# hey-yahei/Quantization.MXNet

Hardware: AMD Instinct MI355X
Metric: images/sec int8-sim MobileNet1.0 (per-layer W8A8, online input quant) (higher is better)
Workload: dtype f32

## Files before the change

### quantization/mxnet_amd/csrc/fq_dw.h

```cpp
#ifndef FQ_DW_H_
#define FQ_DW_H_

#include "fq_common.h"

namespace fqi {

struct DwCall {
  const float *x, *w, *bias;
  float* y;
  int64_t n, c, h, wdt;
  int stride;
  const float *in_stat, *in_thr;
  float* out_current_max;
  const float *bn_scale, *bn_shift;
  int act;
  float* stat_out;
  hipStream_t st;
  bool quant, online, prezeroed;
  int epi;
  float levels, eps;
  int lo_neg;
  int64_t ho, wo;
  void* x_codes_out;
};

bool dw_flat_applies(const DwCall& d, int form), dw_planes_applies(const DwCall& d, int form);
bool dw_cols4_applies(const DwCall& d, int form), dw_cols_applies(const DwCall& d, int form);
bool dw_flat_stat_applies(const DwCall& d);
int dw_run_flat(const DwCall& d), dw_run_planes(const DwCall& d), dw_run_cols4(const DwCall& d), dw_run_cols(const DwCall& d);
int dw_run_tiles(const DwCall& d);
int dw_range_call(const float* x, const float* wcodes_f32, float* y, int64_t n, int64_t c, int64_t h, int64_t wdt, int stride,
                  const float* rec, const float* svec, const float* bn_scale, const float* bn_shift, int act,
                  float* stat_out, hipStream_t st);

}

namespace {

typedef float f2 __attribute__((ext_vector_type(2)));
__device__ __forceinline__ f2 splat2(float v) { return (f2){v, v}; }

__device__ __forceinline__ float dw_taps(float w00, float w01, float w02, float w10, float w11, float w12, float w20,
                                         float w21, float w22, float a0, float a1, float a2, float b0, float b1, float b2,
                                         float c0, float c1, float c2) {
  float acc = 0.0f;
  acc = fmaf(w00, a0, acc);
  acc = fmaf(w01, a1, acc);
  acc = fmaf(w02, a2, acc);
  acc = fmaf(w10, b0, acc);
  acc = fmaf(w11, b1, acc);
  acc = fmaf(w12, b2, acc);
  acc = fmaf(w20, c0, acc);
  acc = fmaf(w21, c1, acc);
  acc = fmaf(w22, c2, acc);
  return acc;
}
__device__ __forceinline__ f2 dw_taps2(float w00, float w01, float w02, float w10, float w11, float w12, float w20, float w21,
                                       float w22, f2 a0, f2 a1, f2 a2, f2 b0, f2 b1, f2 b2, f2 c0, f2 c1, f2 c2) {
  f2 acc = {0.f, 0.f};
  acc = __builtin_elementwise_fma(splat2(w00), a0, acc);
  acc = __builtin_elementwise_fma(splat2(w01), a1, acc);
  acc = __builtin_elementwise_fma(splat2(w02), a2, acc);
  acc = __builtin_elementwise_fma(splat2(w10), b0, acc);
  acc = __builtin_elementwise_fma(splat2(w11), b1, acc);
  acc = __builtin_elementwise_fma(splat2(w12), b2, acc);
  acc = __builtin_elementwise_fma(splat2(w20), c0, acc);
  acc = __builtin_elementwise_fma(splat2(w21), c1, acc);
  acc = __builtin_elementwise_fma(splat2(w22), c2, acc);
  return acc;
}

template <bool ONLINE>
__device__ __forceinline__ QParams dw_qparams(const float* in_stat, int n, const float* in_thr,
                                              float levels, int lo_neg_max, float eps, float* cur_max_out) {
  const float max_ = input_threshold(in_stat, n, ONLINE ? nullptr : in_thr, cur_max_out, blockIdx.x == 0);
  return make_qparams_rt(max_, levels, lo_neg_max, eps, in_thr);
}
template <bool ONLINE>
__device__ __forceinline__ QParams dw_qparams_finish(const ThresholdReq& treq, const float* in_stat, int n,
                                                     const float* in_thr, float levels, int lo_neg_max, float eps,
                                                     float* cur_max_out) {
  const float max_ = threshold_finish(treq, in_stat, n, ONLINE ? nullptr : in_thr, cur_max_out, blockIdx.x == 0);
  return make_qparams_rt(max_, levels, lo_neg_max, eps, in_thr);
}

struct DwBlkRange {
  unsigned begin, end;
  unsigned n_samples;
  unsigned s_base;
};
__device__ __forceinline__ DwBlkRange dw_block_range(unsigned nblk, unsigned tsegs, unsigned segs_per_block, unsigned nsegx,
                                                     unsigned C) {
  DwBlkRange r;
  r.begin = (unsigned)((uint64_t)nblk * blockIdx.x / gridDim.x);
  r.end = (unsigned)((uint64_t)nblk * (blockIdx.x + 1) / gridDim.x);
  r.n_samples = tsegs / nsegx / C;
  const unsigned seg0 = r.begin * segs_per_block;
  r.s_base = (seg0 < tsegs ? seg0 : tsegs - 1) / nsegx / C;
  return r;
}

constexpr int kDwStatSlots = 16;
template <class SampleT>
__device__ __forceinline__ void dw_stat_update(unsigned* k_stat, unsigned s_base, SampleT sample, bool is_out, float m,
                                               int lane, float* stat_out) {
  const unsigned s0 = (unsigned)__builtin_amdgcn_readfirstlane((int)sample);
  const bool wave_uniform = __all(!is_out || (unsigned)sample == s0);
  if (wave_uniform) {
    const float wm = wave_max_nonneg(is_out ? m : 0.0f);
    if (lane == 0 && __float_as_uint(wm) != 0u) {
      const unsigned slot = s0 - s_base;
      if (slot < (unsigned)kDwStatSlots) atomicMax(&k_stat[slot], __float_as_uint(wm));
      else atomic_max_f32(stat_out + s0, wm);
    }
  } else if (is_out) {
    const unsigned slot = (unsigned)sample - s_base;
    if (slot < (unsigned)kDwStatSlots) atomicMax(&k_stat[slot], __float_as_uint(m));
    else atomic_max_f32(stat_out + sample, m);
  }
}
__device__ __forceinline__ void dw_stat_flush(const unsigned* k_stat, unsigned s_base, unsigned n_samples,
                                              float* stat_out) {
  __syncthreads();
  if (threadIdx.x < kDwStatSlots && k_stat[threadIdx.x] != 0u && s_base + threadIdx.x < n_samples)
    FQ_STAT_FLUSH_MAX(reinterpret_cast<unsigned*>(stat_out) + s_base + threadIdx.x, k_stat[threadIdx.x]);
}

__device__ __forceinline__ float keep(float v, bool ok) { return __uint_as_float(__float_as_uint(v) & (ok ? 0xFFFFFFFFu : 0u)); }
__device__ __forceinline__ f4 keep4(f4 v, bool ok) {
  const unsigned mk = ok ? 0xFFFFFFFFu : 0u;
  f4 r;
  r.x = __uint_as_float(__float_as_uint(v.x) & mk);
  r.y = __uint_as_float(__float_as_uint(v.y) & mk);
  r.z = __uint_as_float(__float_as_uint(v.z) & mk);
  r.w = __uint_as_float(__float_as_uint(v.w) & mk);
  return r;
}
__device__ __forceinline__ float left_of(float v, bool first) {
  const float t = lane_prev(v);
  return first ? 0.0f : t;
}
__device__ __forceinline__ float right_of(float v, bool last) {
  const float t = lane_next(v);
  return last ? 0.0f : t;
}

struct DwColGeom {
  int C, H, W, Ho, Wo;
  int sw;
  int nsegx;
  int SEG;
  int segs;
  int nts;
};

__device__ __forceinline__ f2 buf_ld_2f32(fq_rsrc r, unsigned voff, unsigned soff) {
  return __builtin_bit_cast(f2, __builtin_amdgcn_raw_buffer_load_b64(r, (int)voff, (int)soff, 0));
}
__device__ __forceinline__ void buf_st_2f32(fq_rsrc r, unsigned voff, unsigned soff, f2 v) {
  typedef unsigned v2u __attribute__((ext_vector_type(2)));
  __builtin_amdgcn_raw_buffer_store_b64(__builtin_bit_cast(v2u, v), r, (int)voff, (int)soff, 0);
}

constexpr int kEpiRuntime = 0, kEpiBnRelu = 1, kEpiBnRelu6 = 2;
constexpr int kActBiasMul = 0x10;
template <int EPI, bool ACT = true>
__device__ __forceinline__ float dw_finish(float acc, bool has_bias, float bch, bool has_bn, float bsc, float bsh, int act) {
  if (EPI == kEpiRuntime) {
    if (has_bias) acc = (act & kActBiasMul) ? acc * bch : acc + bch;
    if (has_bn) {
      acc = acc * bsc;
      acc = acc + bsh;
    }
    return act_rt(acc, act & 15);
  }
  acc = acc * bsc;
  acc = acc + bsh;
  if (!ACT) return acc;
  acc = fmaxf(acc, 0.0f);
  return EPI == kEpiBnRelu6 ? fminf(acc, 6.0f) : acc;
}
template <int EPI>
__device__ __forceinline__ f2 dw_finish2(f2 acc, bool has_bias, float bch, bool has_bn, float bsc, float bsh, int act) {
  if (EPI == kEpiRuntime) {
    acc.x = dw_finish<EPI>(acc.x, has_bias, bch, has_bn, bsc, bsh, act);
    acc.y = dw_finish<EPI>(acc.y, has_bias, bch, has_bn, bsc, bsh, act);
    return acc;
  }
  acc = acc * splat2(bsc);
  acc = acc + splat2(bsh);
  acc.x = fmaxf(acc.x, 0.0f);
  acc.y = fmaxf(acc.y, 0.0f);
  if (EPI == kEpiBnRelu6) {
    acc.x = fminf(acc.x, 6.0f);
    acc.y = fminf(acc.y, 6.0f);
  }
  return acc;
}

constexpr unsigned kFlagRangeRecord = 0x100u;
constexpr unsigned kFlagBiasMultiplies = 0x200u;

template <class KernelFor, class... Geom>
int dw_launch(const DwCall& d, int grid, size_t lds, KernelFor kernel_for, Geom... geom) {
  using std::integral_constant;
  if (d.stat_out && !d.prezeroed) FQ_HIP(hipMemsetAsync(d.stat_out, 0, d.n * sizeof(float), d.st));
  const double in_bytes = 4.0 * (double)d.n * d.c * d.h * d.wdt, out_bytes = 4.0 * (double)d.n * d.c * d.ho * d.wo;
  ProfScope prof(FQ_KERNEL_DWCONV, in_bytes + out_bytes, d.st,
                 d.y ? -1.0 : in_bytes + (d.x_codes_out ? 0.25 * in_bytes : 0.0));
  float* const y_arg = d.y ? d.y : static_cast<float*>(d.x_codes_out);
  auto launch = [&](auto kernel) {
    hipLaunchKernelGGL(kernel, dim3(grid), dim3(kBlock), lds, d.st, d.x, d.w, d.bias, y_arg, geom..., d.in_stat, (int)d.n,
                       d.in_thr, d.levels, d.lo_neg, d.eps, d.out_current_max, d.bn_scale, d.bn_shift, d.act, d.stat_out);
  };
  auto with_epi = [&](auto quant_c, auto online_c) {
    if (d.epi == kEpiBnRelu) launch(kernel_for(quant_c, online_c, integral_constant<int, kEpiBnRelu>{}));
    else if (d.epi == kEpiBnRelu6) launch(kernel_for(quant_c, online_c, integral_constant<int, kEpiBnRelu6>{}));
    else launch(kernel_for(quant_c, online_c, integral_constant<int, kEpiRuntime>{}));
  };
  if (!d.quant) with_epi(std::false_type{}, std::false_type{});
  else if (d.online) with_epi(std::true_type{}, std::true_type{});
  else with_epi(std::true_type{}, std::false_type{});
  FQ_LAUNCH_CHECK();
  return FQ_OK;
}
template <int V>
using dw_int = std::integral_constant<int, V>;

inline int64_t dw_blocks(int64_t total_segs, int segs) {
  const int64_t per_block = (int64_t)segs * (kBlock / 64);
  return (total_segs + per_block - 1) / per_block;
}
inline int dw_grid(int64_t nblk, int wg_per_cu) {
  const int64_t cap = (int64_t)num_cu() * wg_per_cu;
  return (int)(nblk < cap ? nblk : cap);
}

inline DwColGeom dw_col_geom(const DwCall& d, int units, int halo) {
  DwColGeom cg = {};
  cg.C = (int)d.c;
  cg.H = (int)d.h;
  cg.W = (int)d.wdt;
  cg.Ho = (int)d.ho;
  cg.Wo = (int)d.wo;
  const int max_sw = 64 - halo;
  cg.nsegx = (units + max_sw - 1) / max_sw;
  cg.sw = (units + cg.nsegx - 1) / cg.nsegx;
  cg.SEG = cg.sw + halo;
  cg.segs = 64 / cg.SEG;
  return cg;
}
inline int dw_cols_grid(int64_t total_segs, const DwColGeom& cg) {
  static const int dw_wg_per_cu = env_int("FQ_DW_WG_PER_CU", 6);
  return dw_grid(dw_blocks(total_segs, cg.segs), dw_wg_per_cu);
}

}

#endif
```

### quantization/mxnet_amd/csrc/fq_dw_cols.hip

```cpp
#include "fq_dw.h"

namespace {
template <int S, bool QUANT, bool ONLINE, int EPI>
__global__ __launch_bounds__(kBlock) void dwconv3x3_cols_kernel(
    const float* __restrict__ x, const float* __restrict__ wgt, const float* __restrict__ bias,
    float* __restrict__ y, DwColGeom g, int64_t total_segs, const float* __restrict__ in_stat, int n,
    const float* __restrict__ in_thr, float levels, int lo_neg_max, float eps, float* __restrict__ cur_max_out,
    const float* __restrict__ bn_scale, const float* __restrict__ bn_shift, int act, float* __restrict__ stat_out) {
  constexpr int D = (S == 1) ? 8 : 4;
  __shared__ unsigned k_stat[kDwStatSlots];
  if (threadIdx.x < kDwStatSlots) k_stat[threadIdx.x] = 0u;
  PW_STAMP(0);
  QParams q = {};
  bool q_ready = !QUANT;
  auto ensure_q = [&]() __attribute__((always_inline)) {
    if (QUANT && !q_ready) {
      q = dw_qparams<ONLINE>(in_stat, n, in_thr, levels, lo_neg_max, eps, cur_max_out);
      q_ready = true;
    }
  };
  PW_STAMP(1);
  const int lane = threadIdx.x & 63, wave = threadIdx.x >> 6;
  const int seg_in_wave = lane / g.SEG;
  const int pos = lane - seg_in_wave * g.SEG;
  const bool lane_used = seg_in_wave < g.segs;
  const int64_t segs_per_block = (int64_t)g.segs * (kBlock / 64);
  const int64_t nblk = (total_segs + segs_per_block - 1) / segs_per_block;
  const bool has_bn = bn_scale != nullptr, has_stat = stat_out != nullptr;
  const int plane_in = g.H * g.W, plane_out = g.Ho * g.Wo;

  const unsigned tsegs = (unsigned)total_segs, nsegx = (unsigned)g.nsegx, C_u = (unsigned)g.C;
  const DwBlkRange rg = dw_block_range((unsigned)nblk, tsegs, (unsigned)segs_per_block, nsegx, C_u);
  __syncthreads();
  for (unsigned blk = rg.begin; blk < rg.end; ++blk) {
    const unsigned seg = blk * (unsigned)segs_per_block + (unsigned)wave * (unsigned)g.segs + (unsigned)seg_in_wave;
    const bool seg_ok = lane_used && seg < tsegs;
    const unsigned plane = seg_ok ? seg / nsegx : 0u;
    const int sx = seg_ok ? (int)(seg - plane * nsegx) : 0;
    const unsigned sample_u = plane / C_u;
    const int ch = (int)(plane - sample_u * C_u);
    const int sample = (int)sample_u;
    int oc, ic0;
    bool is_out;
    if (S == 1) {
      ic0 = sx * g.sw + pos - 1;
      oc = ic0;
      is_out = seg_ok && pos >= 1 && pos <= g.sw && oc < g.Wo;
    } else {
      oc = sx * g.sw + pos - 1;
      ic0 = 2 * oc;
      is_out = seg_ok && pos >= 1 && oc < g.Wo;
    }
    const bool ld0 = seg_ok && (S == 1 ? (ic0 >= 0 && ic0 < g.W) : (pos >= 1 && ic0 < g.W));
    const bool ld1 = seg_ok && S == 2 && (ic0 + 1 >= 0) && (ic0 + 1 < g.W);
    const float* xp = x + plane * (int64_t)plane_in + ic0;
    float* yp = y + plane * (int64_t)plane_out + oc;
    const float* wk = wgt + ch * 9;
    const float w00 = wk[0], w01 = wk[1], w02 = wk[2], w10 = wk[3], w11 = wk[4], w12 = wk[5], w20 = wk[6],
                w21 = wk[7], w22 = wk[8];
    const float bch = bias != nullptr ? bias[ch] : 0.0f;
    const float bsc = has_bn ? bn_scale[ch] : 1.0f, bsh = has_bn ? bn_shift[ch] : 0.0f;
    float m = 0.0f;
    if (blk == rg.begin) PW_STAMP(2);

    const int last_row = g.H - 1;
    if (S == 1) {
      const float* xs = ld0 ? xp : x;
      auto ldrow = [&](int row) -> float {
        const int rc = row < last_row ? row : last_row;
        return keep(xs[(int64_t)rc * g.W], ld0 && row <= last_row);
      };
      auto emit = [&](int r, float c1, float& a0, float& a1, float& a2, float& b0, float& b1, float& b2) {
        if (QUANT) c1 = fq_code(c1, q) * q.scale;
        const float c0 = lane_prev(c1), c2 = lane_next(c1);
        float acc = dw_taps(w00, w01, w02, w10, w11, w12, w20, w21, w22, a0, a1, a2, b0, b1, b2, c0, c1, c2);
        acc = dw_finish<EPI>(acc, bias != nullptr, bch, has_bn, bsc, bsh, act);
        m = fmaxf(m, keep(fabsf(acc), is_out));
        if (is_out) yp[(int64_t)r * g.Wo] = acc;
        a0 = b0; a1 = b1; a2 = b2;
        b0 = c0; b1 = c1; b2 = c2;
      };
      float raw[D];
#pragma unroll
      for (int k = 0; k < D; ++k) raw[k] = ldrow(1 + k);
      float a0 = 0.f, a1 = 0.f, a2 = 0.f;
      float b1 = ldrow(0);
      FQ_PIN();
      ensure_q();
      if (QUANT) b1 = fq_code(b1, q) * q.scale;
      float b0 = lane_prev(b1), b2 = lane_next(b1);
      const int rend = g.Ho;
      int r0 = 0;
      for (; r0 + D <= rend; r0 += D) {
#pragma unroll
        for (int k = 0; k < D; ++k) {
          const float c1 = raw[k];
          raw[k] = ldrow(r0 + k + 1 + D);
          emit(r0 + k, c1, a0, a1, a2, b0, b1, b2);
        }
      }
#pragma unroll
      for (int k = 0; k < D; ++k)
        if (r0 + k < rend) emit(r0 + k, raw[k], a0, a1, a2, b0, b1, b2);
    } else {
      const float* xs0 = ld0 ? xp : x;
      const float* xs1 = ld1 ? xp + 1 : x;
      auto ld_a = [&](int row) -> float {
        const int rc = row < last_row ? row : last_row;
        return keep(xs0[(int64_t)rc * g.W], ld0 && row <= last_row);
      };
      auto ld_b = [&](int row) -> float {
        const int rc = row < last_row ? row : last_row;
        return keep(xs1[(int64_t)rc * g.W], ld1 && row <= last_row);
      };
      auto emit2 = [&](int r, float b1, float b2, float c1, float c2, float& a0, float& a1, float& a2) {
        if (QUANT) {
          b1 = fq_code(b1, q) * q.scale;
          b2 = fq_code(b2, q) * q.scale;
          c1 = fq_code(c1, q) * q.scale;
          c2 = fq_code(c2, q) * q.scale;
        }
        const float b0 = lane_prev(b2), c0 = lane_prev(c2);
        float acc = dw_taps(w00, w01, w02, w10, w11, w12, w20, w21, w22, a0, a1, a2, b0, b1, b2, c0, c1, c2);
        acc = dw_finish<EPI>(acc, bias != nullptr, bch, has_bn, bsc, bsh, act);
        m = fmaxf(m, keep(fabsf(acc), is_out));
        if (is_out) yp[(int64_t)r * g.Wo] = acc;
        a0 = c0; a1 = c1; a2 = c2;
      };
      float rb0[D], rb1[D], rc0[D], rc1[D];
#pragma unroll
      for (int k = 0; k < D; ++k) {
        rb0[k] = ld_a(2 * k);
        rb1[k] = ld_b(2 * k);
        rc0[k] = ld_a(2 * k + 1);
        rc1[k] = ld_b(2 * k + 1);
      }
      FQ_PIN();
      ensure_q();
      float a0 = 0.f, a1 = 0.f, a2 = 0.f;
      const int rend = g.Ho;
      int r0 = 0;
      for (; r0 + D <= rend; r0 += D) {
#pragma unroll
        for (int k = 0; k < D; ++k) {
          const float b1 = rb0[k], b2 = rb1[k], c1 = rc0[k], c2 = rc1[k];
          const int rn = r0 + k + D;
          rb0[k] = ld_a(2 * rn);
          rb1[k] = ld_b(2 * rn);
          rc0[k] = ld_a(2 * rn + 1);
          rc1[k] = ld_b(2 * rn + 1);
          emit2(r0 + k, b1, b2, c1, c2, a0, a1, a2);
        }
      }
#pragma unroll
      for (int k = 0; k < D; ++k)
        if (r0 + k < rend) emit2(r0 + k, rb0[k], rb1[k], rc0[k], rc1[k], a0, a1, a2);
    }
    if (blk == rg.begin) PW_STAMP(3);
    if (has_stat) dw_stat_update(k_stat, rg.s_base, sample, is_out, m, lane, stat_out);
  }
  if (has_stat) dw_stat_flush(k_stat, rg.s_base, rg.n_samples, stat_out);
  PW_STAMP(5);
}

template <int S, bool QUANT, bool ONLINE, bool NT, int EPI, bool NOSTORE = false>
__global__ __launch_bounds__(kBlock) void dwconv3x3_cols4_kernel(
    const float* __restrict__ x, const float* __restrict__ wgt, const float* __restrict__ bias,
    float* __restrict__ y, DwColGeom g, int64_t total_segs, const float* __restrict__ in_stat, int n,
    const float* __restrict__ in_thr, float levels, int lo_neg_max, float eps, float* __restrict__ cur_max_out,
    const float* __restrict__ bn_scale, const float* __restrict__ bn_shift, int act, float* __restrict__ stat_out) {
  constexpr int D = (S == 1) ? 4 : 2;
  static_assert(!NOSTORE || (S == 1 && QUANT), "the statistic pass exists for stride 1 with a quantised input");
  __shared__ unsigned k_stat[kDwStatSlots];
  if (threadIdx.x < kDwStatSlots) k_stat[threadIdx.x] = 0u;
  QParams q = {};
  if (QUANT) q = dw_qparams<ONLINE>(in_stat, n, in_thr, levels, lo_neg_max, eps, cur_max_out);
  const int lane = threadIdx.x & 63, wave = threadIdx.x >> 6;
  const int seg_in_wave = lane / g.SEG;
  const int pos = lane - seg_in_wave * g.SEG;
  const bool lane_used = seg_in_wave < g.segs;
  const int64_t segs_per_block = (int64_t)g.segs * (kBlock / 64);
  const int64_t nblk = (total_segs + segs_per_block - 1) / segs_per_block;
  const bool has_bn = bn_scale != nullptr, has_stat = stat_out != nullptr;
  const int plane_in = g.H * g.W, plane_out = g.Ho * g.Wo;
  const int last_row = g.H - 1;
  const unsigned tsegs = (unsigned)total_segs, nsegx = (unsigned)g.nsegx, C_u = (unsigned)g.C;
  const DwBlkRange rg = dw_block_range((unsigned)nblk, tsegs, (unsigned)segs_per_block, nsegx, C_u);
  __syncthreads();
  for (unsigned blk = rg.begin; blk < rg.end; ++blk) {
    const unsigned seg = blk * (unsigned)segs_per_block + (unsigned)wave * (unsigned)g.segs + (unsigned)seg_in_wave;
    const bool seg_ok = lane_used && seg < tsegs;
    const unsigned plane = seg_ok ? seg / nsegx : 0u;
    const int sx = seg_ok ? (int)(seg - plane * nsegx) : 0;
    const unsigned sample_u = plane / C_u;
    const int ch = (int)(plane - sample_u * C_u);
    const int sample = (int)sample_u;
    const int ic0 = (sx * g.sw + pos - 1) * 4;
    const bool ld_ok = seg_ok && ic0 >= 0 && ic0 < g.W;
    const int oc = S == 1 ? ic0 : ic0 / 2;
    const bool is_out = seg_ok && pos >= 1 && pos <= g.sw && oc < g.Wo;
    const f4* xs = reinterpret_cast<const f4*>(ld_ok ? x + plane * (int64_t)plane_in + ic0 : x);
    float* yp = y + plane * (int64_t)plane_out + oc;
    const int rowq = g.W / 4;
    const float* wk = wgt + ch * 9;
    const float w00 = wk[0], w01 = wk[1], w02 = wk[2], w10 = wk[3], w11 = wk[4], w12 = wk[5], w20 = wk[6],
                w21 = wk[7], w22 = wk[8];
    const float bch = bias != nullptr ? bias[ch] : 0.0f;
    const float bsc = has_bn ? bn_scale[ch] : 1.0f, bsh = has_bn ? bn_shift[ch] : 0.0f;
    float m = 0.0f;
    auto ldrow = [&](int row) -> f4 {
      const int rc = row < last_row ? row : last_row;
      return keep4(ld4<NT>(xs + (int64_t)rc * rowq), ld_ok && row <= last_row);
    };
    auto quant4 = [&](f4 v) -> f4 { return QUANT ? fq_code4(v, q) * q.scale : v; };
    auto finish = [&](float acc) -> float { return dw_finish<EPI>(acc, bias != nullptr, bch, has_bn, bsc, bsh, act); };
    unsigned* const cp = reinterpret_cast<unsigned*>(y) + (plane * (int64_t)plane_in + (ld_ok ? ic0 : 0)) / 4;
    auto quant4_keep = [&](f4 v, int row) -> f4 {
      const f4 k = fq_code4(v, q);
      if (y != nullptr && is_out && row <= last_row) {
        const unsigned b0 = (unsigned)(int)k.x & 255u, b1 = (unsigned)(int)k.y & 255u, b2 = (unsigned)(int)k.z & 255u,
                       b3 = (unsigned)(int)k.w & 255u;
        cp[(int64_t)row * rowq] = b0 | (b1 << 8) | (b2 << 16) | (b3 << 24);
      }
      return k * q.scale;
    };

    if (S == 1) {
      float a[6] = {0.f, 0.f, 0.f, 0.f, 0.f, 0.f}, b[6];
      f4 raw[D];
#pragma unroll
      for (int k = 0; k < D; ++k) raw[k] = ldrow(1 + k);
      {
        const f4 v = NOSTORE ? quant4_keep(ldrow(0), 0) : quant4(ldrow(0));
        b[0] = lane_prev(v.w);
        b[1] = v.x; b[2] = v.y; b[3] = v.z; b[4] = v.w;
        b[5] = lane_next(v.x);
      }
      auto emit = [&](int r, f4 craw) {
        const f4 v = NOSTORE ? quant4_keep(craw, r + 1) : quant4(craw);
        float c[6];
        c[0] = lane_prev(v.w);
        c[1] = v.x; c[2] = v.y; c[3] = v.z; c[4] = v.w;
        c[5] = lane_next(v.x);
        float o[4];
#pragma unroll
        for (int k = 0; k < 4; ++k) {
          o[k] = finish(dw_taps(w00, w01, w02, w10, w11, w12, w20, w21, w22, a[k], a[k + 1], a[k + 2], b[k], b[k + 1],
                                b[k + 2], c[k], c[k + 1], c[k + 2]));
        }
        const float mm = fmaxf(fmaxf(fabsf(o[0]), fabsf(o[1])), fmaxf(fabsf(o[2]), fabsf(o[3])));
        m = fmaxf(m, keep(mm, is_out));
        if (!NOSTORE && is_out) {
          if (g.nts) __builtin_nontemporal_store((f4){o[0], o[1], o[2], o[3]}, reinterpret_cast<f4*>(yp + (int64_t)r * g.Wo));
          else *reinterpret_cast<f4*>(yp + (int64_t)r * g.Wo) = (f4){o[0], o[1], o[2], o[3]};
        }
#pragma unroll
        for (int k = 0; k < 6; ++k) {
          a[k] = b[k];
          b[k] = c[k];
        }
      };
      int r0 = 0;
      for (; r0 + D <= g.Ho; r0 += D) {
        f4 nxt[D];
#pragma unroll
        for (int k = 0; k < D; ++k) nxt[k] = ldrow(r0 + k + 1 + D);
#pragma unroll
        for (int k = 0; k < D; ++k) emit(r0 + k, raw[k]);
#pragma unroll
        for (int k = 0; k < D; ++k) raw[k] = nxt[k];
      }
#pragma unroll
      for (int k = 0; k < D; ++k)
        if (r0 + k < g.Ho) emit(r0 + k, raw[k]);
    } else {
      float a[5] = {0.f, 0.f, 0.f, 0.f, 0.f};
      f4 rb[D], rc[D];
#pragma unroll
      for (int k = 0; k < D; ++k) {
        rb[k] = ldrow(2 * k);
        rc[k] = ldrow(2 * k + 1);
      }
      auto emit2 = [&](int r, f4 braw, f4 craw) {
        const f4 vb = quant4(braw), vc = quant4(craw);
        const float b[5] = {lane_prev(vb.w), vb.x, vb.y, vb.z, vb.w};
        const float c[5] = {lane_prev(vc.w), vc.x, vc.y, vc.z, vc.w};
        float o[2];
#pragma unroll
        for (int k = 0; k < 2; ++k) {
          o[k] = finish(dw_taps(w00, w01, w02, w10, w11, w12, w20, w21, w22, a[2 * k], a[2 * k + 1], a[2 * k + 2], b[2 * k],
                                b[2 * k + 1], b[2 * k + 2], c[2 * k], c[2 * k + 1], c[2 * k + 2]));
        }
        m = fmaxf(m, keep(fmaxf(fabsf(o[0]), fabsf(o[1])), is_out));
        if (is_out) {
          typedef float f2v __attribute__((ext_vector_type(2)));
          if (g.nts) __builtin_nontemporal_store((f2v){o[0], o[1]}, reinterpret_cast<f2v*>(yp + (int64_t)r * g.Wo));
          else *reinterpret_cast<float2*>(yp + (int64_t)r * g.Wo) = make_float2(o[0], o[1]);
        }
#pragma unroll
        for (int k = 0; k < 5; ++k) a[k] = c[k];
      };
      int r0 = 0;
      for (; r0 + D <= g.Ho; r0 += D) {
        f4 nb[D], nc[D];
#pragma unroll
        for (int k = 0; k < D; ++k) {
          nb[k] = ldrow(2 * (r0 + k + D));
          nc[k] = ldrow(2 * (r0 + k + D) + 1);
        }
#pragma unroll
        for (int k = 0; k < D; ++k) emit2(r0 + k, rb[k], rc[k]);
#pragma unroll
        for (int k = 0; k < D; ++k) {
          rb[k] = nb[k];
          rc[k] = nc[k];
        }
      }
#pragma unroll
      for (int k = 0; k < D; ++k)
        if (r0 + k < g.Ho) emit2(r0 + k, rb[k], rc[k]);
    }
    if (has_stat) dw_stat_update(k_stat, rg.s_base, sample, is_out, m, lane, stat_out);
  }
  if (has_stat) dw_stat_flush(k_stat, rg.s_base, rg.n_samples, stat_out);
}

}

namespace fqi {
bool dw_cols4_applies(const DwCall& d, int form) {
  const bool can4 = (d.wdt % 4 == 0) && aligned16(d.x) && aligned16(d.y) && aligned16(d.x_codes_out) && ((d.h * d.wdt) % 4 == 0) &&
                    (d.stride == 1 || ((d.wdt / 2) % 2 == 0));
  return (form == 3 || form == 0) && can4;
}
int dw_run_cols4(const DwCall& d) {
  DwColGeom cg = dw_col_geom(d, (int)(d.wdt / 4), d.stride == 1 ? 2 : 1);
  const int64_t total_segs = d.n * d.c * cg.nsegx;
  FQ_REQUIRE(total_segs < (1ll << 31) - 1024, "fq_dwconv3x3: tensor too large for 32-bit segment indices");
  const int grid = dw_cols_grid(total_segs, cg);
  static const int dw_nt_mb = env_int("FQ_DW_NT_MB", 200);
  const bool nt = 4.0 * (double)d.n * d.c * d.h * d.wdt > 1e6 * dw_nt_mb;
  static const int dw_nts_mb = env_int("FQ_DW_NTS_MB", 1 << 30);
  cg.nts = 4.0 * (double)d.n * d.c * cg.Ho * cg.Wo >= 1e6 * dw_nts_mb ? 1 : 0;
  auto go = [&](auto s, auto nt_c) {
    return dw_launch(d, grid, 0, [](auto q, auto o, auto e) {
      return dwconv3x3_cols4_kernel<decltype(s)::value, q(), o(), decltype(nt_c)::value, e()>;
    }, cg, total_segs);
  };
  if (d.y == nullptr) {
    auto go_stat = [&](auto nt_c) {
      return dw_launch(d, grid, 0, [](auto, auto o, auto e) {
        return dwconv3x3_cols4_kernel<1, true, o(), decltype(nt_c)::value, e(), true>;
      }, cg, total_segs);
    };
    return nt ? go_stat(std::true_type{}) : go_stat(std::false_type{});
  }
  if (d.stride == 1) return nt ? go(dw_int<1>{}, std::true_type{}) : go(dw_int<1>{}, std::false_type{});
  return nt ? go(dw_int<2>{}, std::true_type{}) : go(dw_int<2>{}, std::false_type{});
}
bool dw_cols_applies(const DwCall& d, int form) {
  return form == 2 || ((form == 0 || form == 3) && d.wdt >= 14);
}
int dw_run_cols(const DwCall& d) {
  const DwColGeom cg = dw_col_geom(d, (int)d.wo, d.stride == 1 ? 2 : 1);
  const int64_t total_segs = d.n * d.c * cg.nsegx;
  FQ_REQUIRE(total_segs < (1ll << 31) - 1024, "fq_dwconv3x3: tensor too large for 32-bit segment indices");
  const int grid = dw_cols_grid(total_segs, cg);
  auto go = [&](auto s) {
    return dw_launch(d, grid, 0, [](auto q, auto o, auto e) {
      return dwconv3x3_cols_kernel<decltype(s)::value, q(), o(), e()>;
    }, cg, total_segs);
  };
  return d.stride == 1 ? go(dw_int<1>{}) : go(dw_int<2>{});
}
}
```

### quantization/mxnet_amd/csrc/fq_dw_flat.hip

```cpp
#include "fq_dw.h"

namespace {
#define FQ_DWF_PHASE()                                             \
  do {                                                             \
    __builtin_amdgcn_fence(__ATOMIC_RELEASE, "wavefront");         \
    __builtin_amdgcn_wave_barrier();                               \
    __builtin_amdgcn_fence(__ATOMIC_ACQUIRE, "wavefront");         \
  } while (0)

struct DwFlatGeom {
  int C;
  unsigned planes;
  unsigned per, rem;
  FastDiv by_c;
};

template <int S, bool QUANT, bool ONLINE, int H, int W, int EPI>
__global__ __launch_bounds__(kBlock) void dwconv3x3_flat_kernel(
    const float* __restrict__ x, const float* __restrict__ wgt, const float* __restrict__ bias,
    float* __restrict__ y, DwFlatGeom g, const float* __restrict__ in_stat, int n, const float* __restrict__ in_thr,
    float levels, int lo_neg_max, float eps, float* __restrict__ cur_max_out, const float* __restrict__ bn_scale,
    const float* __restrict__ bn_shift, int act, float* __restrict__ stat_out) {
  constexpr bool PAIR = S == 1 && W % 2 == 0, DOWN = S == 2;
  static_assert(S == 1 || W % 2 == 0, "stride 2 reads column pairs");
// ... 117 lines not shown
        }
      } else {
        auto window = [&](float a0, float a1, float a2, float b0, float b1, float b2, float c0, float c1, float c2) -> float {
          float acc = dw_taps(w03.x, w03.y, w03.z, w03.w, w47.x, w47.y, w47.z, w47.w, cur.w8, a0, a1, a2, b0, b1, b2, c0, c1, c2);
          acc = dw_finish<EPI>(acc, has_bias, cur.bch, has_bn, cur.bsc, cur.bsh, act);
          m = fmaxf(m, fabsf(acc));
          return acc;
        };
        if (!DOWN) {
          float* lp = my_tile + j * IN + pos;
          float a0 = 0.f, a1 = 0.f, a2 = 0.f;
          float b1 = lp[0];
          float b0 = left_of(b1, first), b2 = right_of(b1, last);
#pragma unroll
          for (int r = 0; r < H; ++r) {
            float c0 = 0.f, c1 = 0.f, c2 = 0.f;
            if (r + 1 < H) {
              c1 = lp[(r + 1) * W];
              c0 = left_of(c1, first);
              c2 = right_of(c1, last);
            }
            lp[r * W] = window(a0, a1, a2, b0, b1, b2, c0, c1, c2);
            a0 = b0; a1 = b1; a2 = b2;
            b0 = c0; b1 = c1; b2 = c2;
          }
        } else {
          const float* lp = my_tile + j * IN + pos * 2;
          float* op = my_out + j * OUT + pos;
          float a0 = 0.f, a1 = 0.f, a2 = 0.f;
#pragma unroll
          for (int r = 0; r < HO; ++r) {
            const f2 vb = *reinterpret_cast<const f2*>(lp + (2 * r) * W);
            const float b0 = left_of(vb.y, first);
            float c0 = 0.f, c1 = 0.f, c2 = 0.f;
            if (2 * r + 1 < H) {
              const f2 vc = *reinterpret_cast<const f2*>(lp + (2 * r + 1) * W);
              c1 = vc.x;
              c2 = vc.y;
              c0 = left_of(vc.y, first);
            }
            op[r * WO] = window(a0, a1, a2, b0, vb.x, vb.y, c0, c1, c2);
            a0 = c0; a1 = c1; a2 = c2;
          }
        }
      }
    }
    FQ_DWF_PHASE();
    {
      f4 ov[NLO];
#pragma unroll
      for (int i = 0; i < NLO; ++i) ov[i] = DOWN ? otile[wave][lane + 64 * i] : tile[wave][lane + 64 * i];
#pragma unroll
      for (int i = 0; i < NLO; ++i)
        buf_st_v4f_unguarded(ry, (lane + 64u * i) < lim_out ? lane * 16u : kOob, base * (OUT * 4u) + 1024u * i, ov[i]);
      hold_store_data(ov);
    }
    if (has_stat) {
      const unsigned sample = fast_div(base + (is_out ? j : 0u), g.by_c);
      dw_stat_update(k_stat, s_base, sample, is_out, m, (int)lane, stat_out);
    }
    __builtin_amdgcn_wave_barrier();
  }
  PW_STAMP(3);
  if (has_stat) dw_stat_flush(k_stat, s_base, n_samples, stat_out);
  PW_STAMP(5);
}

template <bool ONLINE, int H, int W, int EPI>
__global__ __launch_bounds__(kBlock) void dwconv3x3_flat_stat_kernel(
    const float* __restrict__ x, const float* __restrict__ wgt, const float* __restrict__ bias,
    float* __restrict__ y, DwFlatGeom g, const float* __restrict__ in_stat, int n, const float* __restrict__ in_thr,
    float levels, int lo_neg_max, float eps, float* __restrict__ cur_max_out, const float* __restrict__ bn_scale,
    const float* __restrict__ bn_shift, int act, float* __restrict__ stat_out) {
  static_assert(W % 2 == 0 && (H * W) % 4 == 0, "two columns per lane, planes of whole 16-byte groups");
  constexpr int IN = H * W;
  constexpr int LPP = W / 2;
  constexpr int P = 64 / LPP;
  constexpr int NFI = P * IN / 4;
  constexpr int NLI = (NFI + 63) / 64;
  constexpr unsigned kOob = 0x80000000u;
  __shared__ f4 tile[kBlock / 64][NLI * 64];
  __shared__ unsigned k_stat[kDwStatSlots];
  if (threadIdx.x < kDwStatSlots) k_stat[threadIdx.x] = 0u;
  const unsigned lane = threadIdx.x & 63u;
  const unsigned wave = (unsigned)__builtin_amdgcn_readfirstlane((int)(threadIdx.x >> 6));
  const unsigned b = blockIdx.x;
  const unsigned blk_begin = b * g.per + (b < g.rem ? b : g.rem);
  const unsigned blk_end = blk_begin + g.per + (b < g.rem ? 1u : 0u);
  const unsigned planes = g.planes;
  const unsigned n_samples = (unsigned)n;
  unsigned s_base;
  {
    const unsigned p0 = blk_begin * (P * (kBlock / 64));
    s_base = fast_div(p0 < planes ? p0 : planes - 1, g.by_c);
  }
  const bool has_bn = bn_scale != nullptr, has_stat = stat_out != nullptr, has_bias = bias != nullptr;
  const fq_rsrc rx = make_rsrc(x, (int64_t)planes * IN * 4), rc = make_rsrc(y, y != nullptr ? (int64_t)planes * IN : 0);
  const fq_rsrc rw = make_rsrc(wgt, (int64_t)g.C * 36);
  const unsigned j = lane / LPP, pos = lane - j * LPP;
  const bool b_lane = lane < P * LPP;
  const bool first = pos == 0, last = pos == LPP - 1;
  float* const my_tile = reinterpret_cast<float*>(tile[wave]);

  struct Blk {
    f4 raw[NLI];
    f4 w03, w47;
    float w8, bch, bsc, bsh;
  };
  auto issue = [&](unsigned blk, Blk& k) __attribute__((always_inline)) {
    const unsigned base = (blk * (kBlock / 64) + wave) * P;
    const unsigned left = base < planes ? planes - base : 0u;
    const unsigned np = left < (unsigned)P ? left : (unsigned)P;
    const unsigned lim = np * (IN / 4);
#pragma unroll
    for (int i = 0; i < NLI; ++i)
      k.raw[i] = buf_ld_v4f_nt(rx, (lane + 64u * i) < lim ? lane * 16u : kOob, base * (IN * 4u) + 1024u * i);
    const unsigned ch = (b_lane && j < left) ? fast_mod(base + j, g.by_c) : 0u;
    k.w03 = buf_ld_v4f(rw, ch * 36u, 0);
    k.w47 = buf_ld_v4f(rw, ch * 36u, 16);
    k.w8 = buf_ld_f32(rw, ch * 36u, 32);
    k.bch = has_bias ? bias[ch] : 0.0f;
    k.bsc = has_bn ? bn_scale[ch] : 1.0f;
    k.bsh = has_bn ? bn_shift[ch] : 0.0f;
  };

  Blk nxt;
  const ThresholdReq treq = threshold_request(in_stat, n, ONLINE ? nullptr : in_thr, blockIdx.x == 0);
  FQ_PIN();
  if (blk_begin < blk_end) issue(blk_begin, nxt);
  FQ_PIN();
  const QParams q = dw_qparams_finish<ONLINE>(treq, in_stat, n, in_thr, levels, lo_neg_max, eps, cur_max_out);
  __syncthreads();
  for (unsigned blk = blk_begin; blk < blk_end; ++blk) {
    Blk cur = nxt;
    FQ_PIN();
    if (blk + 1 < blk_end) issue(blk + 1, nxt);
    FQ_PIN();
    const unsigned base = (blk * (kBlock / 64) + wave) * P;
    const unsigned left = base < planes ? planes - base : 0u;
    const unsigned np = left < (unsigned)P ? left : (unsigned)P;
    const unsigned lim = np * (IN / 4);
#pragma unroll
    for (int i = 0; i < NLI; ++i) {
      const f4 k = fq_code4(cur.raw[i], q);
      const unsigned wd = ((unsigned)(int)k.x & 255u) | (((unsigned)(int)k.y & 255u) << 8) | (((unsigned)(int)k.z & 255u) << 16) |
                          (((unsigned)(int)k.w & 255u) << 24);
      buf_st_f32(rc, (lane + 64u * i) < lim ? lane * 4u : kOob, base * (unsigned)IN + 256u * i, __uint_as_float(wd));
      tile[wave][lane + 64 * i] = k * q.scale;
    }
    FQ_DWF_PHASE();
    float m = 0.0f;
    const bool is_out = b_lane && j < left;
    if (b_lane) {
      const f4 w03 = cur.w03, w47 = cur.w47;
      const float* lp = my_tile + j * IN + pos * 2;
      f2 aL = {0.f, 0.f}, aC = {0.f, 0.f}, aR = {0.f, 0.f};
      f2 bL, bC, bR;
      {
        const f2 v = *reinterpret_cast<const f2*>(lp);
        bL = (f2){left_of(v.y, first), v.x};
        bC = v;
        bR = (f2){v.y, right_of(v.x, last)};
      }
#pragma unroll
      for (int r = 0; r < H; ++r) {
        f2 cL = {0.f, 0.f}, cC = {0.f, 0.f}, cR = {0.f, 0.f};
        if (r + 1 < H) {
          const f2 v = *reinterpret_cast<const f2*>(lp + (r + 1) * W);
          cL = (f2){left_of(v.y, first), v.x};
          cC = v;
          cR = (f2){v.y, right_of(v.x, last)};
        }
        f2 acc = dw_taps2(w03.x, w03.y, w03.z, w03.w, w47.x, w47.y, w47.z, w47.w, cur.w8, aL, aC, aR, bL, bC, bR, cL, cC, cR);
        acc = dw_finish2<EPI>(acc, has_bias, cur.bch, has_bn, cur.bsc, cur.bsh, act);
        m = fmaxf(m, fmaxf(fabsf(acc.x), fabsf(acc.y)));
        aL = bL; aC = bC; aR = bR;
        bL = cL; bC = cC; bR = cR;
      }
    }
    if (has_stat) {
      const unsigned sample = fast_div(base + (is_out ? j : 0u), g.by_c);
      dw_stat_update(k_stat, s_base, sample, is_out, m, (int)lane, stat_out);
    }
    FQ_DWF_PHASE();
  }
  if (has_stat) dw_stat_flush(k_stat, s_base, n_samples, stat_out);
}

int dw_flat_kind(const DwCall& d) {
  return (d.h == 14 && d.wdt == 14) ? (d.stride == 1 ? 0 : 1)
         : (d.h == 7 && d.wdt == 7 && d.stride == 1) ? 2
         : (d.h == 28 && d.wdt == 28) ? (d.stride == 1 ? 3 : 4) : -1;
}
int dw_flat_planes(int kind) { return kind == 0 ? 9 : kind >= 3 ? 4 : 8; }

}

namespace fqi {
bool dw_flat_applies(const DwCall& d, int form) {
  static const int flat_on = env_int("FQ_DW_FLAT", 31) & 31;
  const int kind = dw_flat_kind(d);
  const bool whole = kind == 0 || kind >= 3 || (d.n * d.c) % dw_flat_planes(kind) == 0;
  return kind >= 0 && (form == 5 || (form == 0 && ((flat_on >> kind) & 1))) && whole && aligned16(d.x) && aligned16(d.y) &&
         d.n * d.c * d.h * d.wdt * 4 < (1ll << 31);
}
bool dw_flat_stat_applies(const DwCall& d) {
  static const int flat_on = env_int("FQ_DW_FLAT", 31) & 31;
  return d.y == nullptr && d.quant && d.lo_neg != kRangeMode && dw_flat_kind(d) == 3 && ((flat_on >> 3) & 1) && aligned16(d.x) &&
         aligned16(d.x_codes_out) && d.n * d.c * d.h * d.wdt * 4 < (1ll << 31);
}
int dw_run_flat(const DwCall& d) {
  const int kind = dw_flat_kind(d);
  DwFlatGeom fg;
  fg.C = (int)d.c;
  fg.planes = (unsigned)(d.n * d.c);
  fg.by_c = fast_div_for((unsigned)d.c);
  const int64_t nblk = dw_blocks(d.n * d.c, dw_flat_planes(kind));
  static const int fl_tune = env_int("FQ_DW_FLAT_WG_PER_CU", 0);
  const int grid = dw_grid(nblk, fl_tune > 0 ? fl_tune : 3);
  fg.per = (unsigned)(nblk / grid);
  fg.rem = (unsigned)(nblk % grid);
  if (d.y == nullptr)
    return dw_launch(d, grid, 0, [](auto, auto o, auto e) { return dwconv3x3_flat_stat_kernel<o(), 28, 28, e()>; }, fg);
  auto go = [&](auto s, auto hw) {
    return dw_launch(d, grid, 0, [](auto q, auto o, auto e) {
      return dwconv3x3_flat_kernel<decltype(s)::value, q(), o(), decltype(hw)::value, decltype(hw)::value, e()>;
    }, fg);
  };
  return kind == 0 ? go(dw_int<1>{}, dw_int<14>{}) : kind == 1 ? go(dw_int<2>{}, dw_int<14>{})
         : kind == 2 ? go(dw_int<1>{}, dw_int<7>{}) : kind == 4 ? go(dw_int<2>{}, dw_int<28>{})
                     : go(dw_int<1>{}, dw_int<28>{});
}
}
```

Before: 170,100.

## Split depthwise statistic pass into row strips and defer epilogue to min/max

Adds a dedicated statistic kernel for the depthwise conv that only computes the output abs-max. It splits each column block into row strips so small-batch or small-grid layers expose more work units per CU. It also tracks raw accumulator min/max and applies the bias/BN/activation epilogue only to those two values instead of every output, in both the cols and flat kernels. A fast non-negative quantisation path using a reciprocal quotient is added. The costs are halo rows reloaded per strip and reliance on the epilogue being monotonic so the min/max shortcut stays exact.

```diff
diff --git a/quantization/mxnet_amd/csrc/fq_dw.h b/quantization/mxnet_amd/csrc/fq_dw.h
--- a/quantization/mxnet_amd/csrc/fq_dw.h
+++ b/quantization/mxnet_amd/csrc/fq_dw.h
@@ -2,6 +2,7 @@
 #define FQ_DW_H_
 
 #include "fq_common.h"
+#include "fq_dw_strips.h"
 
 namespace fqi {
 
@@ -250,9 +251,23 @@
   cg.segs = 64 / cg.SEG;
   return cg;
 }
+inline int dw_cols_wg_per_cu() {
+  static const int dw_wg_per_cu = env_int("FQ_DW_WG_PER_CU", 6);
+  return dw_wg_per_cu;
+}
 inline int dw_cols_grid(int64_t total_segs, const DwColGeom& cg) {
-  static const int dw_wg_per_cu = env_int("FQ_DW_WG_PER_CU", 6);
-  return dw_grid(dw_blocks(total_segs, cg.segs), dw_wg_per_cu);
+  return dw_grid(dw_blocks(total_segs, cg.segs), dw_cols_wg_per_cu());
+}
+struct DwStatGeom {
+  int strips;
+  FastDiv by_strips;
+};
+inline DwStatGeom dw_stat_geom(int64_t total_segs, const DwColGeom& cg) {
+  const char* e = getenv("FQ_DW_STAT_STRIPS");
+  DwStatGeom sg;
+  sg.strips = dw_stat_strips(dw_blocks(total_segs, cg.segs), cg.H, num_cu(), e != nullptr ? atoi(e) : 0);
+  sg.by_strips = fast_div_for((unsigned)sg.strips);
+  return sg;
 }
 
 }
diff --git a/quantization/mxnet_amd/csrc/fq_dw_cols.hip b/quantization/mxnet_amd/csrc/fq_dw_cols.hip
--- a/quantization/mxnet_amd/csrc/fq_dw_cols.hip
+++ b/quantization/mxnet_amd/csrc/fq_dw_cols.hip
@@ -170,7 +170,7 @@
     const float* __restrict__ in_thr, float levels, int lo_neg_max, float eps, float* __restrict__ cur_max_out,
     const float* __restrict__ bn_scale, const float* __restrict__ bn_shift, int act, float* __restrict__ stat_out) {
   constexpr int D = (S == 1) ? 4 : 2;
-  static_assert(!NOSTORE || (S == 1 && QUANT), "the statistic pass exists for stride 1 with a quantised input");
+  static_assert(!NOSTORE, "the statistic pass is dwconv3x3_cols4_stat_kernel");
   __shared__ unsigned k_stat[kDwStatSlots];
   if (threadIdx.x < kDwStatSlots) k_stat[threadIdx.x] = 0u;
   QParams q = {};
@@ -214,16 +214,6 @@
     };
     auto quant4 = [&](f4 v) -> f4 { return QUANT ? fq_code4(v, q) * q.scale : v; };
     auto finish = [&](float acc) -> float { return dw_finish<EPI>(acc, bias != nullptr, bch, has_bn, bsc, bsh, act); };
-    unsigned* const cp = reinterpret_cast<unsigned*>(y) + (plane * (int64_t)plane_in + (ld_ok ? ic0 : 0)) / 4;
-    auto quant4_keep = [&](f4 v, int row) -> f4 {
-      const f4 k = fq_code4(v, q);
-      if (y != nullptr && is_out && row <= last_row) {
-        const unsigned b0 = (unsigned)(int)k.x & 255u, b1 = (unsigned)(int)k.y & 255u, b2 = (unsigned)(int)k.z & 255u,
-                       b3 = (unsigned)(int)k.w & 255u;
-        cp[(int64_t)row * rowq] = b0 | (b1 << 8) | (b2 << 16) | (b3 << 24);
-      }
-      return k * q.scale;
-    };
 
     if (S == 1) {
       float a[6] = {0.f, 0.f, 0.f, 0.f, 0.f, 0.f}, b[6];
@@ -231,13 +221,13 @@
 #pragma unroll
       for (int k = 0; k < D; ++k) raw[k] = ldrow(1 + k);
       {
-        const f4 v = NOSTORE ? quant4_keep(ldrow(0), 0) : quant4(ldrow(0));
+        const f4 v = quant4(ldrow(0));
         b[0] = lane_prev(v.w);
         b[1] = v.x; b[2] = v.y; b[3] = v.z; b[4] = v.w;
         b[5] = lane_next(v.x);
       }
       auto emit = [&](int r, f4 craw) {
-        const f4 v = NOSTORE ? quant4_keep(craw, r + 1) : quant4(craw);
+        const f4 v = quant4(craw);
         float c[6];
         c[0] = lane_prev(v.w);
         c[1] = v.x; c[2] = v.y; c[3] = v.z; c[4] = v.w;
@@ -250,7 +240,7 @@
         }
         const float mm = fmaxf(fmaxf(fabsf(o[0]), fabsf(o[1])), fmaxf(fabsf(o[2]), fabsf(o[3])));
         m = fmaxf(m, keep(mm, is_out));
-        if (!NOSTORE && is_out) {
+        if (is_out) {
           if (g.nts) __builtin_nontemporal_store((f4){o[0], o[1], o[2], o[3]}, reinterpret_cast<f4*>(yp + (int64_t)r * g.Wo));
           else *reinterpret_cast<f4*>(yp + (int64_t)r * g.Wo) = (f4){o[0], o[1], o[2], o[3]};
         }
@@ -323,6 +313,146 @@
     if (has_stat) dw_stat_update(k_stat, rg.s_base, sample, is_out, m, lane, stat_out);
   }
   if (has_stat) dw_stat_flush(k_stat, rg.s_base, rg.n_samples, stat_out);
+}
+
+template <bool ONLINE, bool NT, int EPI>
+__global__ __launch_bounds__(kBlock) void dwconv3x3_cols4_stat_kernel(
+    const float* __restrict__ x, const float* __restrict__ wgt, const float* __restrict__ bias,
+    float* __restrict__ y, DwColGeom g, int64_t total_segs, DwStatGeom sg, const float* __restrict__ in_stat, int n,
+    const float* __restrict__ in_thr, float levels, int lo_neg_max, float eps, float* __restrict__ cur_max_out,
+    const float* __restrict__ bn_scale, const float* __restrict__ bn_shift, int act, float* __restrict__ stat_out) {
+  constexpr int D = kDwStatBurst;
+  __shared__ unsigned k_stat[kDwStatSlots];
+  if (threadIdx.x < kDwStatSlots) k_stat[threadIdx.x] = 0u;
+  const QParams q = dw_qparams<ONLINE>(in_stat, n, in_thr, levels, lo_neg_max, eps, cur_max_out);
+  const FastQuot fqx = make_fast_quot(q.denom);
+  const bool fast = fq_nonneg(q) && fqx.ok;
+  const int lane = threadIdx.x & 63, wave = threadIdx.x >> 6;
+  const int seg_in_wave = lane / g.SEG;
+  const int pos = lane - seg_in_wave * g.SEG;
+  const bool lane_used = seg_in_wave < g.segs;
+  const unsigned segs_per_block = (unsigned)g.segs * (kBlock / 64);
+  const bool has_bn = bn_scale != nullptr, has_stat = stat_out != nullptr;
+  const int plane_in = g.H * g.W;
+  const int last_row = g.H - 1;
+  const int rowq = g.W / 4;
+  const unsigned tsegs = (unsigned)total_segs, nsegx = (unsigned)g.nsegx, C_u = (unsigned)g.C;
+  const int64_t units = (int64_t)((tsegs + segs_per_block - 1) / segs_per_block) * sg.strips;
+  const unsigned u_begin = (unsigned)dw_stat_unit_begin(units, (int)gridDim.x, (int)blockIdx.x);
+  const unsigned u_end = (unsigned)dw_stat_unit_begin(units, (int)gridDim.x, (int)blockIdx.x + 1);
+  const unsigned n_samples = tsegs / nsegx / C_u;
+  unsigned s_base;
+  {
+    const unsigned seg0 = fast_div(u_begin, sg.by_strips) * segs_per_block;
+    s_base = (seg0 < tsegs ? seg0 : tsegs - 1) / nsegx / C_u;
+  }
+  __syncthreads();
+  auto walk = [&](auto fast_c) __attribute__((always_inline)) {
+    constexpr bool FAST = decltype(fast_c)::value;
+    for (unsigned unit = u_begin; unit < u_end; ++unit) {
+      const unsigned blk = fast_div(unit, sg.by_strips);
+      const DwStrip strip = dw_stat_strip(g.H, sg.strips, (int)(unit - blk * (unsigned)sg.strips));
+      const int r_begin = strip.r0, r_end = strip.r0 + strip.rows;
+      const unsigned seg = blk * segs_per_block + (unsigned)wave * (unsigned)g.segs + (unsigned)seg_in_wave;
+      const bool seg_ok = lane_used && seg < tsegs;
+      const unsigned plane = seg_ok ? seg / nsegx : 0u;
+      const int sx = seg_ok ? (int)(seg - plane * nsegx) : 0;
+      const unsigned sample_u = plane / C_u;
+      const int ch = (int)(plane - sample_u * C_u);
+      const int sample = (int)sample_u;
+      const int ic0 = (sx * g.sw + pos - 1) * 4;
+      const bool ld_ok = seg_ok && ic0 >= 0 && ic0 < g.W;
+      const bool is_out = seg_ok && pos >= 1 && pos <= g.sw && ic0 < g.W;
+      const f4* xs = reinterpret_cast<const f4*>(ld_ok ? x + plane * (int64_t)plane_in + ic0 : x);
+      const float* wk = wgt + ch * 9;
+      const float w00 = wk[0], w01 = wk[1], w02 = wk[2], w10 = wk[3], w11 = wk[4], w12 = wk[5], w20 = wk[6],
+                  w21 = wk[7], w22 = wk[8];
+      const float bch = bias != nullptr ? bias[ch] : 0.0f;
+      const float bsc = has_bn ? bn_scale[ch] : 1.0f, bsh = has_bn ? bn_shift[ch] : 0.0f;
+      const int row_hi = r_end < last_row ? r_end : last_row;
+      auto ldrow = [&](int row) -> f4 {
+        const int rc = row < 0 ? 0 : (row < row_hi ? row : row_hi);
+        return keep4(ld4<NT>(xs + (int64_t)rc * rowq), ld_ok && row >= 0 && row <= last_row);
+      };
+      unsigned* const cp = reinterpret_cast<unsigned*>(y) + (plane * (int64_t)plane_in + (ld_ok ? ic0 : 0)) / 4;
+      const bool keeps = y != nullptr && is_out;
+      auto quant_row = [&](f4 v, int row, bool own) -> f4 {
+        if (FAST) {
+          const int k0 = fq_code_nonneg(v.x, q, fqx), k1 = fq_code_nonneg(v.y, q, fqx), k2 = fq_code_nonneg(v.z, q, fqx),
+                    k3 = fq_code_nonneg(v.w, q, fqx);
+          if (keeps && own)
+            cp[(int64_t)row * rowq] = (unsigned)k0 | ((unsigned)k1 << 8) | ((unsigned)k2 << 16) | ((unsigned)k3 << 24);
+          return (f4){(float)k0, (float)k1, (float)k2, (float)k3} * q.scale;
+        }
+        const f4 k = fq_code4(v, q);
+        if (keeps && own) {
+          const unsigned b0 = (unsigned)(int)k.x & 255u, b1 = (unsigned)(int)k.y & 255u, b2 = (unsigned)(int)k.z & 255u,
+                         b3 = (unsigned)(int)k.w & 255u;
+          cp[(int64_t)row * rowq] = b0 | (b1 << 8) | (b2 << 16) | (b3 << 24);
+        }
+        return k * q.scale;
+      };
+      auto window_row = [&](f4 v, float (&t)[6]) {
+        t[0] = lane_prev(v.w);
+        t[1] = v.x; t[2] = v.y; t[3] = v.z; t[4] = v.w;
+        t[5] = lane_next(v.x);
+      };
+
+      float a[6], b[6];
+      f4 raw[D];
+#pragma unroll
+      for (int k = 0; k < D; ++k) raw[k] = ldrow(r_begin + 1 + k);
+      {
+        const f4 above = ldrow(r_begin - 1), first = ldrow(r_begin);
+        window_row(quant_row(above, r_begin - 1, false), a);
+        window_row(quant_row(first, r_begin, true), b);
+      }
+      float mx = -INFINITY, mn = INFINITY;
+      auto emit = [&](int r, f4 craw) {
+        float c[6];
+        window_row(quant_row(craw, r + 1, r + 1 < r_end), c);
+#pragma unroll
+        for (int k = 0; k < 4; k += 2) {
+          const float o0 = dw_taps(w00, w01, w02, w10, w11, w12, w20, w21, w22, a[k], a[k + 1], a[k + 2], b[k], b[k + 1],
+                                   b[k + 2], c[k], c[k + 1], c[k + 2]);
+          const float o1 = dw_taps(w00, w01, w02, w10, w11, w12, w20, w21, w22, a[k + 1], a[k + 2], a[k + 3], b[k + 1], b[k + 2],
+                                   b[k + 3], c[k + 1], c[k + 2], c[k + 3]);
+          mx = fmaxf(fmaxf(mx, o0), o1);
+          mn = fminf(fminf(mn, o0), o1);
+        }
+#pragma unroll
+        for (int k = 0; k < 6; ++k) {
+          a[k] = b[k];
+          b[k] = c[k];
+        }
+      };
+      int r0 = r_begin;
+      for (; r0 + D <= r_end; r0 += D) {
+        f4 nxt[D];
+#pragma unroll
+        for (int k = 0; k < D; ++k) nxt[k] = ldrow(r0 + k + 1 + D);
+#pragma unroll
+        for (int k = 0; k < D; ++k) emit(r0 + k, raw[k]);
+#pragma unroll
+        for (int k = 0; k < D; ++k) raw[k] = nxt[k];
+      }
+#pragma unroll
+      for (int k = 0; k < D; ++k)
+        if (r0 + k < r_end) emit(r0 + k, raw[k]);
+      if (has_stat) {
+        float m = 0.0f;
+        if (mx >= mn) {
+          const float at_max = dw_finish<EPI>(mx, bias != nullptr, bch, has_bn, bsc, bsh, act);
+          const float at_min = dw_finish<EPI>(mn, bias != nullptr, bch, has_bn, bsc, bsh, act);
+          m = fmaxf(fmaxf(0.0f, fabsf(at_max)), fabsf(at_min));
+        }
+        dw_stat_update(k_stat, s_base, sample, is_out, m, lane, stat_out);
+      }
+    }
+  };
+  if (fast) walk(std::true_type{});
+  else walk(std::false_type{});
+  if (has_stat) dw_stat_flush(k_stat, s_base, n_samples, stat_out);
 }
 
 }
@@ -348,10 +478,14 @@
     }, cg, total_segs);
   };
   if (d.y == nullptr) {
+    const DwStatGeom sg = dw_stat_geom(total_segs, cg);
+    const int64_t nblk = dw_blocks(total_segs, cg.segs);
+    FQ_REQUIRE(nblk * sg.strips < (1ll << 31), "fq_dwconv3x3: tensor too large for 32-bit strip indices");
+    const int stat_grid = dw_stat_grid(nblk, sg.strips, num_cu(), dw_cols_wg_per_cu());
     auto go_stat = [&](auto nt_c) {
-      return dw_launch(d, grid, 0, [](auto, auto o, auto e) {
-        return dwconv3x3_cols4_kernel<1, true, o(), decltype(nt_c)::value, e(), true>;
-      }, cg, total_segs);
+      return dw_launch(d, stat_grid, 0, [](auto, auto o, auto e) {
+        return dwconv3x3_cols4_stat_kernel<o(), decltype(nt_c)::value, e()>;
+      }, cg, total_segs, sg);
     };
     return nt ? go_stat(std::true_type{}) : go_stat(std::false_type{});
   }
diff --git a/quantization/mxnet_amd/csrc/fq_dw_flat.hip b/quantization/mxnet_amd/csrc/fq_dw_flat.hip
--- a/quantization/mxnet_amd/csrc/fq_dw_flat.hip
+++ b/quantization/mxnet_amd/csrc/fq_dw_flat.hip
@@ -293,6 +293,7 @@
     float m = 0.0f;
     const bool is_out = b_lane && j < left;
     if (b_lane) {
+      float mx = -INFINITY, mn = INFINITY;
       const f4 w03 = cur.w03, w47 = cur.w47;
       const float* lp = my_tile + j * IN + pos * 2;
       f2 aL = {0.f, 0.f}, aC = {0.f, 0.f}, aR = {0.f, 0.f};
@@ -312,11 +313,15 @@
           cC = v;
           cR = (f2){v.y, right_of(v.x, last)};
         }
-        f2 acc = dw_taps2(w03.x, w03.y, w03.z, w03.w, w47.x, w47.y, w47.z, w47.w, cur.w8, aL, aC, aR, bL, bC, bR, cL, cC, cR);
-        acc = dw_finish2<EPI>(acc, has_bias, cur.bch, has_bn, cur.bsc, cur.bsh, act);
-        m = fmaxf(m, fmaxf(fabsf(acc.x), fabsf(acc.y)));
+        const f2 acc = dw_taps2(w03.x, w03.y, w03.z, w03.w, w47.x, w47.y, w47.z, w47.w, cur.w8, aL, aC, aR, bL, bC, bR, cL, cC, cR);
+        mx = fmaxf(fmaxf(mx, acc.x), acc.y);
+        mn = fminf(fminf(mn, acc.x), acc.y);
         aL = bL; aC = bC; aR = bR;
         bL = cL; bC = cC; bR = cR;
+      }
+      if (mx >= mn) {
+        const f2 e = dw_finish2<EPI>((f2){mx, mn}, has_bias, cur.bch, has_bn, cur.bsc, cur.bsh, act);
+        m = fmaxf(fmaxf(0.0f, fabsf(e.x)), fabsf(e.y));
       }
     }
     if (has_stat) {
diff --git a/quantization/mxnet_amd/csrc/fq_dw_strips.h b/quantization/mxnet_amd/csrc/fq_dw_strips.h
--- /dev/null
+++ b/quantization/mxnet_amd/csrc/fq_dw_strips.h
@@ -0,0 +1,35 @@
+#ifndef FQ_DW_STRIPS_H_
+#define FQ_DW_STRIPS_H_
+
+#include <cstdint>
+
+namespace fqi {
+
+constexpr int kDwStatBurst = 4;
+constexpr int kDwStatWavesPerSimd = 4;
+constexpr int kDwStatWavesPerWg = 4, kDwStatSimdsPerCu = 4;
+
+struct DwStrip {
+  int r0, rows;
+};
+constexpr DwStrip dw_stat_strip(int h, int strips, int s) {
+  const int base = h / strips, rem = h % strips;
+  return DwStrip{s * base + (s < rem ? s : rem), base + (s < rem ? 1 : 0)};
+}
+constexpr int dw_stat_strips(int64_t nblk, int h, int cus, int forced) {
+  if (forced > 0) return forced < h ? forced : h;
+  const int64_t want = (int64_t)cus * kDwStatSimdsPerCu * kDwStatWavesPerSimd / kDwStatWavesPerWg;
+  int64_t s = nblk > 0 ? (want + nblk - 1) / nblk : 1;
+  const int64_t most = h / kDwStatBurst;
+  if (s > most) s = most;
+  return s < 1 ? 1 : (int)s;
+}
+constexpr int dw_stat_grid(int64_t nblk, int strips, int cus, int wg_per_cu) {
+  const int64_t units = nblk * strips, cap = (int64_t)cus * wg_per_cu;
+  return (int)(units < cap ? units : cap);
+}
+constexpr int64_t dw_stat_unit_begin(int64_t units, int grid, int b) { return units * b / grid; }
+
+}
+
+#endif
```

Measured after the change: 170,400 (median of 2 runs). Within noise of the previous version (+0.2%).
